# andreaskoepf/faster-rcnn.torch

Hardware: AMD Instinct MI355X
Metric: images/sec (vgg_small 800x450 fwd+bwd) (higher is better)
Workload: dtype f32 (conv / Linear(13824,1024) operands as 2 x fp16 split planes: 22 significand bits, 3 MFMA partial products; fp32 accumulate)

## Files before the change

### faster-rcnn.torch_amd/csrc/gemm.hip

```cpp
#include <cstdlib>
#include "kernels.h"

namespace frcnn {

typedef float f32x16 __attribute__((ext_vector_type(16)));

#define GB 64
#ifndef GBK
#define GBK 32
#endif

struct GemmGroup { GemmJob job[GEMM_GROUP_MAX]; int start[GEMM_GROUP_MAX + 1]; int tm[GEMM_GROUP_MAX], tn[GEMM_GROUP_MAX]; int n; };

struct GemmArgs {
  const float* A; long sAm, sAk;
  const float* B; long sBk, sBn;
  float* C; long ldc;
  const float* bias;
  int M, N, K, kPerSplit, out_mode;
};

__device__ __forceinline__ void gemm_store_tile(const f32x16& a, const GemmArgs& p, int mb, int n, int split) {
  const bool nok = n < p.N;
  const int nc = min(n, p.N - 1);
  const float bv = (p.bias && split == 0) ? p.bias[nc] : 0.f;
  float* const col = (p.out_mode == 3 ? p.C + (long)split * p.M * p.N : p.C) + nc;
  const long rs = p.out_mode == 3 ? (long)p.N : p.ldc;
  if (p.out_mode == 1) {
    float old[16];
#pragma unroll
    for (int r = 0; r < 16; ++r) old[r] = col[(long)min(mb + (r & 3) + 8 * (r >> 2), p.M - 1) * rs];
#pragma unroll
    for (int r = 0; r < 16; ++r) {
      const int m = mb + (r & 3) + 8 * (r >> 2);
      if (nok && m < p.M) col[(long)m * rs] = old[r] + (a[r] + bv);
    }
  } else {
#pragma unroll
    for (int r = 0; r < 16; ++r) {
      const int m = mb + (r & 3) + 8 * (r >> 2);
      if (nok && m < p.M) col[(long)m * rs] = a[r] + bv;
    }
  }
}


template <int ROWS, bool KC, bool VEC>
struct TileLoader {
  static constexpr int NV = ROWS * GBK / 1024;
  static constexpr int NS = ROWS * GBK / 256;
  static constexpr int PITCH = ROWS + 1;
  float4 v4[NV];
  float v1[VEC ? 1 : NS];
  __device__ __forceinline__ static void coord_v(int tid, int it, int& r, int& k) {
    if (KC) { k = (tid % (GBK / 4)) * 4; r = tid / (GBK / 4) + (1024 / GBK) * it; }
    else    { r = (tid % (ROWS / 4)) * 4; k = tid / (ROWS / 4) + (1024 / ROWS) * it; }
  }
  __device__ __forceinline__ static void coord_s(int tid, int it, int& r, int& k) {
    if (KC) { k = tid % GBK; r = tid / GBK + (256 / GBK) * it; }
    else    { r = tid % ROWS; k = tid / ROWS + (256 / ROWS) * it; }
  }
  __device__ __forceinline__ void load(const float* __restrict__ P, long sRow, long sK, int row0, int nRows, int k0,
                                       int kEnd, int tid) {
    if (VEC) {
#pragma unroll
      for (int it = 0; it < NV; ++it) {
        int r, k;
        coord_v(tid, it, r, k);
        const int rr = min(row0 + r, nRows - (KC ? 1 : 4)), kk = min(k0 + k, kEnd - (KC ? 4 : 1));
        v4[it] = *reinterpret_cast<const float4*>(P + (long)rr * sRow + (long)kk * sK);
      }
    } else {
#pragma unroll
      for (int it = 0; it < NS; ++it) {
        int r, k;
        coord_s(tid, it, r, k);
        const int rr = min(row0 + r, nRows - 1), kk = min(k0 + k, kEnd - 1);
        v1[it] = P[(long)rr * sRow + (long)kk * sK];
      }
    }
  }
  __device__ __forceinline__ void store(float* __restrict__ T, int row0, int nRows, int k0, int kEnd, int tid) {
    if (VEC) {
#pragma unroll
      for (int it = 0; it < NV; ++it) {
        int r, k;
        coord_v(tid, it, r, k);
        const float e[4] = {v4[it].x, v4[it].y, v4[it].z, v4[it].w};
#pragma unroll
        for (int j = 0; j < 4; ++j) {
          const int rj = KC ? r : r + j, kj = KC ? k + j : k;
          T[kj * PITCH + rj] = (row0 + rj < nRows && k0 + kj < kEnd) ? e[j] : 0.f;
        }
      }
    } else {
#pragma unroll
      for (int it = 0; it < NS; ++it) {
        int r, k;
        coord_s(tid, it, r, k);
        T[k * PITCH + r] = (row0 + r < nRows && k0 + k < kEnd) ? v1[it] : 0.f;
      }
    }
  }
};

template <int TM, int TN, bool AK, bool BK_, bool AV, bool BV>
__device__ __forceinline__ void gemm_tile(const GemmArgs& p, int bx, int by, int bz, float* As, float* Bs) {
  constexpr int PA = TM + 1, PB = TN + 1, MT = TM / 64, NT = TN / 64;
  const int tid = threadIdx.x, lane = tid & 63, wave = tid >> 6;
  const int wm = wave >> 1, wn = wave & 1, h = lane >> 5, li = lane & 31;
  const int m0 = by * TM, n0 = bx * TN;
  const int kbeg = bz * p.kPerSplit;
  const int kend = min(kbeg + p.kPerSplit, p.K);
  f32x16 acc[MT][NT];
#pragma unroll
  for (int a = 0; a < MT; ++a)
#pragma unroll
    for (int b = 0; b < NT; ++b)
#pragma unroll
      for (int r = 0; r < 16; ++r) acc[a][b][r] = 0.f;
  TileLoader<TM, AK, AV> la;
  TileLoader<TN, BK_, BV> lb;

  for (int k0 = kbeg; k0 < kend; k0 += GBK) {
    la.load(p.A, p.sAm, p.sAk, m0, p.M, k0, kend, tid);
    lb.load(p.B, p.sBn, p.sBk, n0, p.N, k0, kend, tid);
    la.store(As, m0, p.M, k0, kend, tid);
    lb.store(Bs, n0, p.N, k0, kend, tid);
    __syncthreads();
#pragma unroll
    for (int kk = 0; kk < GBK / 2; ++kk) {
      float a[MT], b[NT];
#pragma unroll
      for (int i = 0; i < MT; ++i) a[i] = As[(kk * 2 + h) * PA + wm * (TM / 2) + i * 32 + li];
#pragma unroll
      for (int j = 0; j < NT; ++j) b[j] = Bs[(kk * 2 + h) * PB + wn * (TN / 2) + j * 32 + li];
#pragma unroll
      for (int i = 0; i < MT; ++i)
#pragma unroll
        for (int j = 0; j < NT; ++j) acc[i][j] = __builtin_amdgcn_mfma_f32_32x32x2f32(a[i], b[j], acc[i][j], 0, 0, 0);
    }
    __syncthreads();
  }
#pragma unroll
  for (int j = 0; j < NT; ++j) {
    const int n = n0 + wn * (TN / 2) + j * 32 + li;
#pragma unroll
    for (int i = 0; i < MT; ++i)
      gemm_store_tile(acc[i][j], p, m0 + wm * (TM / 2) + i * 32 + 4 * h, n, bz);
  }
}

template <int TM, int TN, bool AK, bool BK_, bool AV, bool BV>
__global__ __launch_bounds__(256) void gemm_kernel(GemmArgs p) {
  __shared__ float As[GBK * (TM + 1)];
  __shared__ float Bs[GBK * (TN + 1)];
  gemm_tile<TM, TN, AK, BK_, AV, BV>(p, blockIdx.x, blockIdx.y, blockIdx.z, As, Bs);
}

template <bool AK, bool BK_>
__global__ __launch_bounds__(256) void gemm_group_kernel(GemmGroup g) {
  __shared__ float As[GBK * (GB + 1)];
  __shared__ float Bs[GBK * (GB + 1)];
  int j = 0;
  while (j + 1 < g.n && (int)blockIdx.x >= g.start[j + 1]) ++j;
  const int b = blockIdx.x - g.start[j];
  const int tiles = g.tn[j] * g.tm[j];
  const int bz = b / tiles, r = b - bz * tiles;
  GemmArgs p;
  const GemmJob& q = g.job[j];
  p.A = q.A; p.sAm = q.sAm; p.sAk = q.sAk; p.B = q.B; p.sBk = q.sBk; p.sBn = q.sBn; p.C = q.C; p.ldc = q.ldc; p.bias = nullptr;
  p.M = q.M; p.N = q.N; p.K = q.K; p.kPerSplit = q.kPerSplit; p.out_mode = q.out_mode;
  gemm_tile<GB, GB, AK, BK_, false, false>(p, r % g.tn[j], r / g.tn[j], bz, As, Bs);
}

#ifndef GD_BK
#define GD_BK 32
#endif
#ifndef GD_STAGES
#define GD_STAGES 1
#endif
__device__ __attribute__((aligned(16))) float g_zero16[4] = {0.f, 0.f, 0.f, 0.f};

template <int ROWS, bool KCONT>
__device__ __forceinline__ void gd_issue(const float* __restrict__ P, long sRow, long sK, int row0, int nRows, int k0,
                                         int kend, float* lds, int wave_u, int lane) {
  constexpr int NINST = ROWS * GD_BK / 256;
#pragma unroll
  for (int j = 0; j < NINST / 4; ++j) {
    const int inst = wave_u + 4 * j;
    const int slot = inst * 64 + lane;
    const float* src;
    if (KCONT) {
      const int r = slot / (GD_BK / 4), cphys = slot % (GD_BK / 4);
      const int k = k0 + ((cphys ^ (r & 7)) << 2);
      const int rr = min(row0 + r, nRows - 1);
      src = k < kend ? P + (long)rr * sRow + k : g_zero16;
    } else {
      const int kr = slot / (ROWS / 4), r4 = (slot % (ROWS / 4)) * 4;
      const int k = k0 + kr;
      const int rr = min(row0 + r4, nRows - 4);
      src = k < kend ? P + (long)k * sK + rr : g_zero16;
    }
    __builtin_amdgcn_global_load_lds((const __attribute__((address_space(1))) void*)src,
                                     (__attribute__((address_space(3))) void*)(lds + inst * 256), 16, 0, 0);
  }
}

template <int TM, int TN, bool AK, bool BK_>
__global__ __launch_bounds__(256) void gemm_dma_kernel(GemmArgs p) {
  constexpr int MT = TM / 64, NT = TN / 64;
  constexpr int AF = TM * GD_BK, BF = TN * GD_BK;
  extern __shared__ __attribute__((aligned(16))) float gsm[];
  float* As = gsm;
  float* Bs = gsm + GD_STAGES * AF;
  const int tid = threadIdx.x, lane = tid & 63;
  const int wave = __builtin_amdgcn_readfirstlane(tid >> 6);
  const int wm = wave >> 1, wn = wave & 1, h = lane >> 5, li = lane & 31;
  const int m0 = blockIdx.y * TM, n0 = blockIdx.x * TN;
  const int kbeg = blockIdx.z * p.kPerSplit;
  const int kend = min(kbeg + p.kPerSplit, p.K);
  f32x16 acc[MT][NT];
#pragma unroll
  for (int a = 0; a < MT; ++a)
#pragma unroll
    for (int b = 0; b < NT; ++b)
#pragma unroll
      for (int r = 0; r < 16; ++r) acc[a][b][r] = 0.f;

  auto stage = [&](int k0, int buf) {
    gd_issue<TM, AK>(p.A, p.sAm, p.sAk, m0, p.M, k0, kend, As + buf * AF, wave, lane);
    gd_issue<TN, BK_>(p.B, p.sBn, p.sBk, n0, p.N, k0, kend, Bs + buf * BF, wave, lane);
  };
#define GD_DMA_WAIT() asm volatile("s_waitcnt vmcnt(0)" ::: "memory")
  if (GD_STAGES == 2) stage(kbeg, 0);
  GD_DMA_WAIT();
  __syncthreads();
  int cur = 0;
  for (int k0 = kbeg; k0 < kend; k0 += GD_BK) {
    if (GD_STAGES == 2) {
      if (k0 + GD_BK < kend) stage(k0 + GD_BK, cur ^ 1);
    } else {
      stage(k0, 0);
      GD_DMA_WAIT();
      __syncthreads();
    }
    const float* A_ = As + cur * AF;
    const float* B_ = Bs + cur * BF;
#pragma unroll
    for (int g = 0; g < GD_BK / 8; ++g) {
      float a[MT][4], b[NT][4];
#pragma unroll
      for (int mt = 0; mt < MT; ++mt) {
        const int arow = wm * (TM / 2) + mt * 32 + li;
        if (AK) {
          const float4 v = *reinterpret_cast<const float4*>(A_ + (arow * (GD_BK / 4) + ((2 * g + h) ^ (arow & 7))) * 4);
          a[mt][0] = v.x; a[mt][1] = v.y; a[mt][2] = v.z; a[mt][3] = v.w;
        } else {
#pragma unroll
          for (int j = 0; j < 4; ++j) a[mt][j] = A_[(8 * g + 4 * h + j) * TM + arow];
        }
      }
#pragma unroll
      for (int nt = 0; nt < NT; ++nt) {
        const int brow = wn * (TN / 2) + nt * 32 + li;
        if (BK_) {
          const float4 v = *reinterpret_cast<const float4*>(B_ + (brow * (GD_BK / 4) + ((2 * g + h) ^ (brow & 7))) * 4);
          b[nt][0] = v.x; b[nt][1] = v.y; b[nt][2] = v.z; b[nt][3] = v.w;
        } else {
#pragma unroll
          for (int j = 0; j < 4; ++j) b[nt][j] = B_[(8 * g + 4 * h + j) * TN + brow];
        }
      }
#pragma unroll
      for (int j = 0; j < 4; ++j)
#pragma unroll
        for (int mt = 0; mt < MT; ++mt)
#pragma unroll
          for (int nt = 0; nt < NT; ++nt)
            acc[mt][nt] = __builtin_amdgcn_mfma_f32_32x32x2f32(a[mt][j], b[nt][j], acc[mt][nt], 0, 0, 0);
    }
    if (GD_STAGES == 2) GD_DMA_WAIT();
    __syncthreads();
    if (GD_STAGES == 2) cur ^= 1;
  }
#pragma unroll
  for (int j = 0; j < NT; ++j) {
    const int n = n0 + wn * (TN / 2) + j * 32 + li;
#pragma unroll
    for (int i = 0; i < MT; ++i)
      gemm_store_tile(acc[i][j], p, m0 + wm * (TM / 2) + i * 32 + 4 * h, n, (int)blockIdx.z);
  }
}

__global__ void gemm_reduce_kernel(const float* __restrict__ slab, int nSplit, int M, int N, const float* __restrict__ bias,
                                   float* __restrict__ C, long ldc, int accumulate) {
  const long total = (long)M * N;
  for (long t = (long)blockIdx.x * blockDim.x + threadIdx.x; t < total; t += (long)gridDim.x * blockDim.x) {
    const int m = (int)(t / N), n = (int)(t - (long)m * N);
    float v = bias ? bias[n] : 0.f;
    for (int sI = 0; sI < nSplit; ++sI) v += slab[(size_t)sI * total + t];
    float* dst = C + (long)m * ldc + n;
    if (accumulate) *dst += v; else *dst = v;
  }
}

static void* g_gemm_ws[8] = {};
static size_t g_gemm_ws_bytes[8] = {};
static int gemm_workspace(size_t need, float** out, int slot) {
  if (need > g_gemm_ws_bytes[slot]) {
    if (g_gemm_ws[slot]) FR_HIP(hipFree(g_gemm_ws[slot]));
    g_gemm_ws[slot] = nullptr; g_gemm_ws_bytes[slot] = 0;
    FR_HIP(hipMalloc(&g_gemm_ws[slot], need));
    g_gemm_ws_bytes[slot] = need;
  }
  *out = (float*)g_gemm_ws[slot];
  return FRCNN_OK;
}

int gemm_workspace_get(size_t need, float** out, int slot) { return gemm_workspace(need, out, slot); }
int gemm_reduce_slabs(const float* slab, int nSplit, int M, int N, const float* bias, float* C, long ldc, bool accumulate,
                      hipStream_t s) {
  const long total = (long)M * N;
  const int rgrid = (int)std::min<long>(cdivl(total, 256), 2048);
  FR_LAUNCH(KC_ELEMWISE, 0, total * 4.0 * (nSplit + 1), s, gemm_reduce_kernel, dim3(rgrid), dim3(256), 0, slab, nSplit, M, N, bias,
            C, ldc, accumulate ? 1 : 0);
  FR_LAUNCH_CHECK();
  return FRCNN_OK;
}

int gemm_f32(const float* A, long sAm, long sAk, const float* B, long sBk, long sBn, float* C,
             long ldc, int M, int N, int K, int out_mode, const float* bias_n, hipStream_t s, int ws_slot, GemmFold* defer) {
  if (defer) *defer = GemmFold{};
  if (M <= 0 || N <= 0) return FRCNN_OK;
  GemmArgs p;
  p.A = A; p.sAm = sAm; p.sAk = sAk; p.B = B; p.sBk = sBk; p.sBn = sBn; p.C = C; p.ldc = ldc;
  p.bias = bias_n; p.M = M; p.N = N; p.K = K;
  constexpr int TMs = 64;
  const int TNs = (N >= 2048 && K >= 512) ? 128 : 64;
  int tm = cdiv(M, TMs), tn = cdiv(N, TNs);
  long tiles = (long)tm * tn;
  const long slots = TNs == 128 ? 1280 : 2048;
  int splitK = (int)std::max<long>(1, std::min<long>(std::min<long>(K / 256, 16), slots / tiles));
  p.kPerSplit = cdiv(cdiv(K, splitK), GBK) * GBK;
  splitK = cdiv(K, p.kPerSplit);
  p.out_mode = out_mode;
  float* user_C = C;
  if (splitK > 1) {
    float* ws = nullptr;
    FR_TRY(gemm_workspace((size_t)splitK * M * N * 4, &ws, ws_slot & 7));
    p.C = ws; p.bias = nullptr; p.out_mode = 3;
  }
  dim3 grid(tn, tm, splitK);
  double flops = 2.0 * M * N * (double)K;
  double bytes = 4.0 * ((double)M * K + (double)K * N + (double)M * N);
  const bool ak = sAk == 1, bk = sBk == 1;
  auto vec_ok = [](const float* P, bool kc, long sRow, long sK, int nRows, int Kdim, int kPer) {
    if (((uintptr_t)P & 15) != 0) return false;
    if (kc) return sK == 1 && (sRow % 4) == 0 && (Kdim % 4) == 0 && (kPer % 4) == 0;
    return sRow == 1 && (sK % 4) == 0 && (nRows % 4) == 0;
  };
  const bool av = vec_ok(A, ak, sAm, sAk, M, K, p.kPerSplit), bv = vec_ok(B, bk, sBn, sBk, N, K, p.kPerSplit);
  auto chunk_ok = [](const float* P, bool kc, long sRow, long sK, int nRows, int Kdim, int kPer) {
    if (((uintptr_t)P & 3) != 0) return false;
    if (kc) return sK == 1 && (Kdim % 4) == 0 && (kPer % 4) == 0;
    return sRow == 1 && (nRows % 4) == 0;
  };
  const bool ad = chunk_ok(A, ak, sAm, sAk, M, K, p.kPerSplit);
  const bool bd = chunk_ok(B, bk, sBn, sBk, N, K, p.kPerSplit);
  const bool dma_ok = ad && bd && (p.kPerSplit % GD_BK == 0 || splitK == 1) && K >= 64 &&
                      (ak ? true : (M % 4 == 0 && M >= 4)) && (bk ? true : (N % 4 == 0 && N >= 4));
  if (dma_ok) {
    const size_t lds = (size_t)GD_STAGES * (TMs + TNs) * GD_BK * 4;
#define GEMM_DMA(TMv, TNv, AKv, BKv)                                                                              \
  do {                                                                                                            \
    static bool attr_ = false;                                                                                    \
    if (!attr_) {                                                                                                 \
      FR_HIP(hipFuncSetAttribute(reinterpret_cast<const void*>(gemm_dma_kernel<TMv, TNv, AKv, BKv>),              \
                                 hipFuncAttributeMaxDynamicSharedMemorySize, 160 * 1024));                        \
      attr_ = true;                                                                                               \
    }                                                                                                             \
    FR_LAUNCH(KC_GEMM, flops, bytes, s, (gemm_dma_kernel<TMv, TNv, AKv, BKv>), grid, dim3(256), lds, p);          \
  } while (0)
#define GEMM_DMA_T(TMv, TNv)                                                       \
  do {                                                                             \
    if (ak && bk) GEMM_DMA(TMv, TNv, true, true);                                  \
    else if (ak) GEMM_DMA(TMv, TNv, true, false);                                  \
    else if (bk) GEMM_DMA(TMv, TNv, false, true);                                  \
    else GEMM_DMA(TMv, TNv, false, false);                                         \
  } while (0)
    if (TNs == 128) GEMM_DMA_T(TMs, 128);
    else GEMM_DMA_T(TMs, 64);
#undef GEMM_DMA_T
#undef GEMM_DMA
  } else {
  const int sel = (ak ? 8 : 0) | (bk ? 4 : 0) | (av ? 2 : 0) | (bv ? 1 : 0);
#define GEMM_LAUNCH(TMv, TNv, AKv, BKv, AVv, BVv) \
  FR_LAUNCH(KC_GEMM, flops, bytes, s, (gemm_kernel<TMv, TNv, AKv, BKv, AVv, BVv>), grid, dim3(256), 0, p)
#define GEMM_CASE(AKv, BKv, AVv, BVv)                                                                        \
  case ((AKv ? 8 : 0) | (BKv ? 4 : 0) | (AVv ? 2 : 0) | (BVv ? 1 : 0)):                                      \
    if (TNs == 128) GEMM_LAUNCH(TMs, 128, AKv, BKv, AVv, BVv);                                               \
    else GEMM_LAUNCH(TMs, 64, AKv, BKv, AVv, BVv);                                                           \
    break;
  switch (sel) {
    GEMM_CASE(true, true, true, true) GEMM_CASE(true, true, true, false) GEMM_CASE(true, true, false, true)
    GEMM_CASE(true, true, false, false) GEMM_CASE(true, false, true, true) GEMM_CASE(true, false, true, false)
    GEMM_CASE(true, false, false, true) GEMM_CASE(true, false, false, false) GEMM_CASE(false, true, true, true)
    GEMM_CASE(false, true, true, false) GEMM_CASE(false, true, false, true) GEMM_CASE(false, true, false, false)
    GEMM_CASE(false, false, true, true) GEMM_CASE(false, false, true, false) GEMM_CASE(false, false, false, true)
    GEMM_CASE(false, false, false, false)
  }
#undef GEMM_CASE
#undef GEMM_LAUNCH
  }
  if (splitK > 1 && splitK <= 8 && defer && out_mode == OUT_STORE && ldc == N) {
    defer->slab = p.C; defer->nSplit = splitK; defer->bias = bias_n;
  } else if (splitK > 1) {
    long total = (long)M * N;
    int rgrid = (int)std::min<long>(cdivl(total, 256), 2048);
    FR_LAUNCH(KC_ELEMWISE, 0, total * 4.0 * (splitK + 1), s, gemm_reduce_kernel, dim3(rgrid), dim3(256), 0, (const float*)p.C,
              splitK, M, N, bias_n, user_C, ldc, out_mode == OUT_ADD ? 1 : 0);
  }
  FR_LAUNCH_CHECK();
  return FRCNN_OK;
}

int gemm_f32_group(GemmJob* jobs, int n, hipStream_t s) {
  FR_CHECK(n >= 1 && n <= GEMM_GROUP_MAX, "gemm_f32_group: %d jobs", n);
  GemmGroup g;
  g.n = n;
  int at = 0;
  double flops = 0, bytes = 0;
  const bool ak = jobs[0].sAk == 1, bk = jobs[0].sBk == 1;
  for (int j = 0; j < n; ++j) {
    GemmJob& q = jobs[j];
    const int splits = std::max(1, q.splits);
    q.kPerSplit = cdiv(cdiv(q.K, splits), GBK) * GBK;
    const int ns = (q.M > 0 && q.N > 0) ? cdiv(q.K, q.kPerSplit) : 0;
    if (splits > 1) { FR_CHECK(ns == splits, "gemm_f32_group: %d splits of K = %d leave one empty", splits, q.K); q.out_mode = 3; }
    g.job[j] = q;
    g.tm[j] = cdiv(q.M, GB); g.tn[j] = cdiv(q.N, GB);
    g.start[j] = at;
    at += g.tm[j] * g.tn[j] * ns;
    flops += 2.0 * q.M * q.N * (double)q.K;
    bytes += 4.0 * ((double)q.M * q.K + (double)q.K * q.N + (double)q.M * q.N);
  }
  g.start[n] = at;
  if (at == 0) return FRCNN_OK;
  if (ak && bk) FR_LAUNCH(KC_GEMM, flops, bytes, s, (gemm_group_kernel<true, true>), dim3(at), dim3(256), 0, g);
  else if (ak) FR_LAUNCH(KC_GEMM, flops, bytes, s, (gemm_group_kernel<true, false>), dim3(at), dim3(256), 0, g);
  else if (bk) FR_LAUNCH(KC_GEMM, flops, bytes, s, (gemm_group_kernel<false, true>), dim3(at), dim3(256), 0, g);
  else FR_LAUNCH(KC_GEMM, flops, bytes, s, (gemm_group_kernel<false, false>), dim3(at), dim3(256), 0, g);
  FR_LAUNCH_CHECK();
  return FRCNN_OK;
}

}
```

### faster-rcnn.torch_amd/csrc/roi.hip

```cpp
#include "kernels.h"
#include "roi_fix.h"

namespace frcnn {

__global__ void roi_pool_forward_kernel(const float* __restrict__ fmap, int C, int H, int W,
                                        const int* __restrict__ wins, int R, int kh, int kw,
                                        float* __restrict__ out, int* __restrict__ idx) {
  const long total = (long)R * C * kh * kw;
  for (long t = (long)blockIdx.x * blockDim.x + threadIdx.x; t < total; t += (long)gridDim.x * blockDim.x) {
    int j = (int)(t % kw);
    long q = t / kw;
    int i = (int)(q % kh);
    q /= kh;
    int c = (int)(q % C);
    int r = (int)(q / C);
    const int* wn = wins + 4 * r;
    const int r0 = wn[0] - 1, c0 = wn[2] - 1;
    const int h = wn[1] - wn[0] + 1, w = wn[3] - wn[2] + 1;
    const int ys = (i * h) / kh, ye = ((i + 1) * h + kh - 1) / kh;
    const int xs = (j * w) / kw, xe = ((j + 1) * w + kw - 1) / kw;
    const float* ip = fmap + (size_t)c * H * W;
    float best = -3.402823466e+38f;
    int bi = -1;
    for (int y = ys; y < ye; ++y)
      for (int x = xs; x < xe; ++x) {
        float v = ip[(size_t)(r0 + y) * W + (c0 + x)];
        if (v > best) { best = v; bi = (r0 + y) * W + (c0 + x); }
      }
    out[t] = best;
    if (idx) idx[t] = bi;
  }
}

__global__ __launch_bounds__(256) void roi_pool_forward_cells_kernel(const float* __restrict__ fmap, int C, int H, int W,
                                                                     const int* __restrict__ wins, int kh, int kw,
                                                                     float* __restrict__ out, int* __restrict__ idx) {
  const int r = blockIdx.x, cells = kh * kw, groups = blockDim.x / cells;
  const int tid = threadIdx.x;
  if (tid >= groups * cells) return;
  const int cg = tid / cells, cell = tid - cg * cells;
  const int i = cell / kw, j = cell - i * kw;
  const int* wn = wins + 4 * r;
  const int r0 = wn[0] - 1, c0 = wn[2] - 1;
  const int h = wn[1] - wn[0] + 1, w = wn[3] - wn[2] + 1;
  const int ys = (i * h) / kh, ye = ((i + 1) * h + kh - 1) / kh;
  const int xs = (j * w) / kw, xe = ((j + 1) * w + kw - 1) / kw;
  const int HW = H * W;
  const int base = (r0 + ys) * W + c0 + xs, nx = xe - xs, ny = ye - ys;
  if (HW >= 4) {
    for (int c = blockIdx.y * groups + cg; c < C; c += gridDim.y * groups) {
      const float* ip = fmap + (size_t)c * HW;
      float best = -3.402823466e+38f;
      int bi = -1;
      for (int y = 0, o = base; y < ny; ++y, o += W)
        for (int x = 0; x < nx; x += 4) {
          const int q = min(o + x, HW - 4);
          float v[4];
          __builtin_memcpy(v, ip + q, 16);
#pragma unroll
          for (int e = 0; e < 4; ++e) {
            const int at = q + e;
            if (at >= o && at < o + nx && v[e] > best) { best = v[e]; bi = at; }
          }
        }
      const size_t t = ((size_t)r * C + c) * cells + cell;
      out[t] = best;
      if (idx) idx[t] = bi;
    }
    return;
  }
  for (int c = blockIdx.y * groups + cg; c < C; c += gridDim.y * groups) {
    const float* ip = fmap + (size_t)c * HW;
    float best = -3.402823466e+38f;
    int bi = -1;
    for (int y = 0, o = base; y < ny; ++y, o += W)
      for (int x = 0; x < nx; ++x) {
        const float v = ip[o + x];
        if (v > best) { best = v; bi = o + x; }
      }
    const size_t t = ((size_t)r * C + c) * cells + cell;
    out[t] = best;
    if (idx) idx[t] = bi;
  }
}

int roi_pool_forward(const float* fmap, int C, int H, int W, const int* wins, int R, int kh, int kw,
                     float* out, int* idx, hipStream_t s) {
  if (R <= 0) return FRCNN_OK;
  long total = (long)R * C * kh * kw;
  if (kh * kw <= 256) {
    const int groups = 256 / (kh * kw);
    const int slices = std::max(1, std::min(cdiv(C, groups), (int)cdivl(4096, R)));
    FR_LAUNCH(KC_ROI, 0, total * 8.0, s, roi_pool_forward_cells_kernel, dim3(R, slices), dim3(256), 0, fmap, C, H, W,
              wins, kh, kw, out, idx);
    FR_LAUNCH_CHECK();
    return FRCNN_OK;
  }
  int grid = (int)std::min<long>(cdivl(total, 256), 4096);
  FR_LAUNCH(KC_ROI, 0, total * 8.0, s, roi_pool_forward_kernel, dim3(grid), dim3(256), 0, fmap, C, H, W,
            wins, R, kh, kw, out, idx);
  FR_LAUNCH_CHECK();
  return FRCNN_OK;
}

__global__ void roi_pool_backward_lds_kernel(float* __restrict__ gmap, int C, int HW, const float* __restrict__ gout,
                                             const int* __restrict__ idx, int R, int cell) {
  extern __shared__ float plane[];
  const int c = blockIdx.x;
  for (int i = threadIdx.x; i < HW; i += blockDim.x) plane[i] = 0.f;
  __syncthreads();
  const long D = (long)C * cell;
  const int total = R * cell;
  for (int e = threadIdx.x; e < total; e += blockDim.x) {
    const int r = e / cell, j = e - r * cell;
    const long t = (long)r * D + (long)c * cell + j;
    const int bi = idx[t];
    const float g = gout[t];
    if (bi >= 0 && g != 0.f) atomicAdd(&plane[bi], g);
  }
  __syncthreads();
  float* gp = gmap + (size_t)c * HW;
  for (int i = threadIdx.x; i < HW; i += blockDim.x) {
    const float v = plane[i];
    if (v != 0.f) gp[i] += v;
  }
}

__global__ void roi_pool_backward_lds_det_kernel(float* __restrict__ gmap, int C, int HW, const float* __restrict__ gout,
                                                 const int* __restrict__ idx, int R, int cell) {
  extern __shared__ unsigned long long fplane[];
  const int c = blockIdx.x;
  for (int i = threadIdx.x; i < HW; i += blockDim.x) fplane[i] = 0ull;
  __syncthreads();
  const long D = (long)C * cell;
  const int total = R * cell;
  for (int e = threadIdx.x; e < total; e += blockDim.x) {
    const int r = e / cell, j = e - r * cell;
    const long t = (long)r * D + (long)c * cell + j;
    const int bi = idx[t];
    const float g = gout[t];
    if (bi >= 0 && g != 0.f) atomicAdd(&fplane[bi], (unsigned long long)roi_to_fix(g));
  }
  __syncthreads();
  float* gp = gmap + (size_t)c * HW;
  for (int i = threadIdx.x; i < HW; i += blockDim.x) {
    const long long v = (long long)fplane[i];
    if (v != 0) gp[i] += (float)((double)v / ROI_FIX_SCALE);
  }
}
__global__ void roi_pool_backward_det_kernel(unsigned long long* __restrict__ fix, int C, long HW,
                                             const float* __restrict__ gout, const int* __restrict__ idx,
                                             long total, int cell) {
  for (long t = (long)blockIdx.x * blockDim.x + threadIdx.x; t < total; t += (long)gridDim.x * blockDim.x) {
    int c = (int)((t / cell) % C);
    int bi = idx[t];
    float g = gout[t];
    if (bi >= 0 && g != 0.f) atomicAdd(fix + (size_t)c * HW + bi, (unsigned long long)roi_to_fix(g));
  }
}
__global__ void roi_fix_apply_kernel(const unsigned long long* __restrict__ fix, long n, float* __restrict__ gmap) {
  for (long t = (long)blockIdx.x * blockDim.x + threadIdx.x; t < n; t += (long)gridDim.x * blockDim.x) {
    const long long v = (long long)fix[t];
    if (v != 0) gmap[t] += (float)((double)v / ROI_FIX_SCALE);
  }
}

int roi_fix_apply(const unsigned long long* fix, long n, float* gmap, hipStream_t s) {
  FR_LAUNCH(KC_ROI, 0, n * 16.0, s, roi_fix_apply_kernel, dim3((int)std::min<long>(cdivl(n, 256), 4096)), dim3(256), 0, fix, n, gmap);
  FR_LAUNCH_CHECK();
  return FRCNN_OK;
}

__global__ void roi_pool_backward_kernel(float* __restrict__ gmap, int C, long HW,
                                         const float* __restrict__ gout, const int* __restrict__ idx,
                                         long total, int cell) {
  for (long t = (long)blockIdx.x * blockDim.x + threadIdx.x; t < total; t += (long)gridDim.x * blockDim.x) {
    int c = (int)((t / cell) % C);
    int bi = idx[t];
    float g = gout[t];
    if (bi >= 0 && g != 0.f) unsafeAtomicAdd(gmap + (size_t)c * HW + bi, g);
  }
}

int roi_pool_backward(float* gmap, int C, int H, int W, const float* gout, const int* idx, int R,
                      int kh, int kw, hipStream_t s) {
  if (R <= 0) return FRCNN_OK;
  long total = (long)R * C * kh * kw;
  if (deterministic()) {
    if ((size_t)H * W * 8 <= 64 * 1024) {
      FR_LAUNCH(KC_ROI, 0, total * 12.0, s, roi_pool_backward_lds_det_kernel, dim3(C), dim3(256), (size_t)H * W * 8, gmap, C,
                H * W, gout, idx, R, kh * kw);
    } else {
      float* ws = nullptr;
      const long n = (long)C * H * W;
      FR_TRY(det_workspace(s, (size_t)n * 2, &ws));
      FR_HIP(hipMemsetAsync(ws, 0, (size_t)n * 8, s));
      int grid = (int)std::min<long>(cdivl(total, 256), 4096);
      FR_LAUNCH(KC_ROI, 0, total * 12.0, s, roi_pool_backward_det_kernel, dim3(grid), dim3(256), 0, (unsigned long long*)ws, C,
                (long)H * W, gout, idx, total, kh * kw);
      FR_LAUNCH_CHECK();
      return roi_fix_apply((const unsigned long long*)ws, n, gmap, s);
    }
    FR_LAUNCH_CHECK();
    return FRCNN_OK;
  }
  if ((size_t)H * W * 4 <= 64 * 1024) {
    FR_LAUNCH(KC_ROI, 0, total * 12.0, s, roi_pool_backward_lds_kernel, dim3(C), dim3(1024), (size_t)H * W * 4, gmap, C,
              H * W, gout, idx, R, kh * kw);
    FR_LAUNCH_CHECK();
    return FRCNN_OK;
  }
  int grid = (int)std::min<long>(cdivl(total, 256), 4096);
  FR_LAUNCH(KC_ROI, 0, total * 12.0, s, roi_pool_backward_kernel, dim3(grid), dim3(256), 0, gmap, C,
            (long)H * W, gout, idx, total, kh * kw);
  FR_LAUNCH_CHECK();
  return FRCNN_OK;
}

}
```

Before: 520.1.

## Vectorize split-K reduction and stage ROI-pool feature planes in LDS

```diff
diff --git a/faster-rcnn.torch_amd/csrc/gemm.hip b/faster-rcnn.torch_amd/csrc/gemm.hip
--- a/faster-rcnn.torch_amd/csrc/gemm.hip
+++ b/faster-rcnn.torch_amd/csrc/gemm.hip
@@ -293,16 +293,45 @@
   }
 }
 
-__global__ void gemm_reduce_kernel(const float* __restrict__ slab, int nSplit, int M, int N, const float* __restrict__ bias,
-                                   float* __restrict__ C, long ldc, int accumulate) {
-  const long total = (long)M * N;
-  for (long t = (long)blockIdx.x * blockDim.x + threadIdx.x; t < total; t += (long)gridDim.x * blockDim.x) {
-    const int m = (int)(t / N), n = (int)(t - (long)m * N);
-    float v = bias ? bias[n] : 0.f;
-    for (int sI = 0; sI < nSplit; ++sI) v += slab[(size_t)sI * total + t];
-    float* dst = C + (long)m * ldc + n;
-    if (accumulate) *dst += v; else *dst = v;
-  }
+__device__ __forceinline__ float4 gr_add(float4 a, float4 b) { return make_float4(a.x + b.x, a.y + b.y, a.z + b.z, a.w + b.w); }
+__device__ __forceinline__ float gr_add(float a, float b) { return a + b; }
+__device__ __forceinline__ void gr_zero(float4& v) { v = make_float4(0.f, 0.f, 0.f, 0.f); }
+__device__ __forceinline__ void gr_zero(float& v) { v = 0.f; }
+template <class V>
+__global__ __launch_bounds__(256) void gemm_reduce_kernel(const float* __restrict__ slab, int nSplit, int M, int N,
+                                                          const float* __restrict__ bias, float* __restrict__ C, long ldc,
+                                                          int accumulate) {
+  constexpr int E = sizeof(V) / 4;
+  const int Nv = N / E;
+  const long total = (long)M * Nv, stride = (long)gridDim.x * blockDim.x;
+  const long ldv = ldc / E;
+  const V* __restrict__ sv = reinterpret_cast<const V*>(slab);
+  const V* __restrict__ bv = reinterpret_cast<const V*>(bias);
+  V* __restrict__ cv = reinterpret_cast<V*>(C);
+  long t = (long)blockIdx.x * blockDim.x + threadIdx.x;
+  if (t >= total) return;
+  long m = t / Nv;
+  int n = (int)(t - m * Nv);
+  const long dm = stride / Nv;
+  const int dn = (int)(stride - dm * Nv);
+  for (; t < total; t += stride) {
+    V v;
+    if (bias) v = bv[n]; else gr_zero(v);
+    int sI = 0;
+    const V* p = sv + t;
+    for (; sI + 4 <= nSplit; sI += 4, p += 4 * total) {
+      const V a = p[0], b = p[total], c = p[2 * total], d = p[3 * total];
+      v = gr_add(gr_add(gr_add(gr_add(v, a), b), c), d);
+    }
+    for (; sI < nSplit; ++sI, p += total) v = gr_add(v, *p);
+    V* dst = cv + m * ldv + n;
+    *dst = accumulate ? gr_add(*dst, v) : v;
+    n += dn; m += dm;
+    if (n >= Nv) { n -= Nv; ++m; }
+  }
+}
+static bool gemm_reduce_vec_ok(const float* slab, int N, const float* bias, const float* C, long ldc) {
+  return N % 4 == 0 && ldc % 4 == 0 && (((uintptr_t)slab | (uintptr_t)bias | (uintptr_t)C) & 15) == 0;
 }
 
 static void* g_gemm_ws[8] = {};
@@ -322,9 +351,15 @@
 int gemm_reduce_slabs(const float* slab, int nSplit, int M, int N, const float* bias, float* C, long ldc, bool accumulate,
                       hipStream_t s) {
   const long total = (long)M * N;
-  const int rgrid = (int)std::min<long>(cdivl(total, 256), 2048);
-  FR_LAUNCH(KC_ELEMWISE, 0, total * 4.0 * (nSplit + 1), s, gemm_reduce_kernel, dim3(rgrid), dim3(256), 0, slab, nSplit, M, N, bias,
-            C, ldc, accumulate ? 1 : 0);
+  if (gemm_reduce_vec_ok(slab, N, bias, C, ldc)) {
+    const int rgrid = (int)std::min<long>(cdivl(total / 4, 256), 2048);
+    FR_LAUNCH(KC_ELEMWISE, 0, total * 4.0 * (nSplit + 1), s, gemm_reduce_kernel<float4>, dim3(rgrid), dim3(256), 0, slab, nSplit, M, N,
+              bias, C, ldc, accumulate ? 1 : 0);
+  } else {
+    const int rgrid = (int)std::min<long>(cdivl(total, 256), 2048);
+    FR_LAUNCH(KC_ELEMWISE, 0, total * 4.0 * (nSplit + 1), s, gemm_reduce_kernel<float>, dim3(rgrid), dim3(256), 0, slab, nSplit, M, N,
+              bias, C, ldc, accumulate ? 1 : 0);
+  }
   FR_LAUNCH_CHECK();
   return FRCNN_OK;
 }
@@ -416,10 +451,7 @@
   if (splitK > 1 && splitK <= 8 && defer && out_mode == OUT_STORE && ldc == N) {
     defer->slab = p.C; defer->nSplit = splitK; defer->bias = bias_n;
   } else if (splitK > 1) {
-    long total = (long)M * N;
-    int rgrid = (int)std::min<long>(cdivl(total, 256), 2048);
-    FR_LAUNCH(KC_ELEMWISE, 0, total * 4.0 * (splitK + 1), s, gemm_reduce_kernel, dim3(rgrid), dim3(256), 0, (const float*)p.C,
-              splitK, M, N, bias_n, user_C, ldc, out_mode == OUT_ADD ? 1 : 0);
+    FR_TRY(gemm_reduce_slabs(p.C, splitK, M, N, bias_n, user_C, ldc, out_mode == OUT_ADD, s));
   }
   FR_LAUNCH_CHECK();
   return FRCNN_OK;
diff --git a/faster-rcnn.torch_amd/csrc/roi.hip b/faster-rcnn.torch_amd/csrc/roi.hip
--- a/faster-rcnn.torch_amd/csrc/roi.hip
+++ b/faster-rcnn.torch_amd/csrc/roi.hip
@@ -84,10 +84,101 @@
   }
 }
 
+#define ROI_FWD_THREADS 512
+#define ROI_FWD_TAB 1024
+#define ROI_FWD_TAB_BYTES ((ROI_FWD_TAB + 256) * 4)
+__global__ __launch_bounds__(ROI_FWD_THREADS) void roi_pool_forward_lds_kernel(const float* __restrict__ fmap, int C, int H, int W,
+                                                                               const int* __restrict__ wins, int R, int kh, int kw,
+                                                                               int G, int rois_per_block, float* __restrict__ out,
+                                                                               int* __restrict__ idx) {
+  extern __shared__ __attribute__((aligned(16))) unsigned char roi_smem[];
+  int* const tab = reinterpret_cast<int*>(roi_smem);
+  int* const celltab = tab + ROI_FWD_TAB;
+  float* const planes = reinterpret_cast<float*>(roi_smem + ROI_FWD_TAB_BYTES);
+  const int tid = threadIdx.x, B = blockDim.x;
+  const int HW = H * W, cells = kh * kw, kk = kh + kw;
+  const int c0 = blockIdx.x * G, Gc = min(G, C - c0);
+  const int r_begin = blockIdx.y * rois_per_block, r_end = min(R, r_begin + rois_per_block);
+  {
+    const float* __restrict__ src = fmap + (size_t)c0 * HW;
+    const int n = Gc * HW;
+    int head = (int)(((16 - (reinterpret_cast<uintptr_t>(src) & 15)) & 15) >> 2);
+    if (head > n) head = n;
+    const int n4 = (n - head) >> 2;
+    const float4* __restrict__ s4 = reinterpret_cast<const float4*>(src + head);
+    for (int e = tid; e < n4; e += B) {
+      const float4 v = s4[e];
+      float* d = planes + head + 4 * e;
+      d[0] = v.x; d[1] = v.y; d[2] = v.z; d[3] = v.w;
+    }
+    if (tid < head) planes[tid] = src[tid];
+    if (head + 4 * n4 + tid < n) planes[head + 4 * n4 + tid] = src[head + 4 * n4 + tid];
+  }
+  if (tid < cells) { const int i = tid / kw; celltab[tid] = i | ((tid - i * kw) << 16); }
+  const int chunk = ROI_FWD_TAB / kk;
+  int* const ytab = tab;
+  int* const xtab = tab + chunk * kh;
+  const int d_cell = B % cells, bq = B / cells, d_cl = bq % Gc, d_rl = bq / Gc;
+  for (int rc = r_begin; rc < r_end; rc += chunk) {
+    const int nr = min(chunk, r_end - rc);
+    __syncthreads();
+    for (int e = tid; e < nr * kk; e += B) {
+      const int rl = e / kk, k = e - rl * kk;
+      const int* wn = wins + 4 * (rc + rl);
+      if (k < kh) {
+        const int r0 = wn[0] - 1, h = wn[1] - wn[0] + 1;
+        ytab[rl * kh + k] = (r0 + (k * h) / kh) | ((r0 + ((k + 1) * h + kh - 1) / kh) << 16);
+      } else {
+        const int j = k - kh, x0 = wn[2] - 1, w = wn[3] - wn[2] + 1;
+        xtab[rl * kw + j] = (x0 + (j * w) / kw) | ((x0 + ((j + 1) * w + kw - 1) / kw) << 16);
+      }
+    }
+    __syncthreads();
+    const int items = nr * Gc * cells;
+    int cell = tid % cells, q = tid / cells;
+    int cl = q % Gc, rl = q / Gc;
+    for (int t = tid; t < items; t += B) {
+      const int ij = celltab[cell], i = ij & 0xFFFF, j = ij >> 16;
+      const int yb = ytab[rl * kh + i], xb = xtab[rl * kw + j];
+      const int y0 = yb & 0xFFFF, y1 = yb >> 16, x0 = xb & 0xFFFF, x1 = xb >> 16;
+      const float* pl = planes + cl * HW;
+      float best = -3.402823466e+38f;
+      int bi = -1;
+      for (int y = y0, o = y0 * W; y < y1; ++y, o += W)
+        for (int x = x0; x < x1; ++x) {
+          const float v = pl[o + x];
+          if (v > best) { best = v; bi = o + x; }
+        }
+      const size_t at = ((size_t)(rc + rl) * C + c0 + cl) * cells + cell;
+      out[at] = best;
+      if (idx) idx[at] = bi;
+      cell += d_cell;
+      const int carry = cell >= cells;
+      cell -= carry ? cells : 0;
+      cl += d_cl + carry;
+      const int carry2 = cl >= Gc;
+      cl -= carry2 ? Gc : 0;
+      rl += d_rl + carry2;
+    }
+  }
+}
+
 int roi_pool_forward(const float* fmap, int C, int H, int W, const int* wins, int R, int kh, int kw,
                      float* out, int* idx, hipStream_t s) {
   if (R <= 0) return FRCNN_OK;
   long total = (long)R * C * kh * kw;
+  if (kh * kw <= 256 && H * W >= 4 && H <= 32767 && W <= 32767 && (size_t)H * W * 4 + ROI_FWD_TAB_BYTES <= 64 * 1024) {
+    const size_t plane = (size_t)H * W * 4;
+    int G = (int)std::max<size_t>(1, std::min<size_t>((size_t)C, (40 * 1024) / plane));
+    const int ngroups = cdiv(C, G);
+    G = cdiv(C, ngroups);
+    const int rpb = cdiv(R, std::max(1, std::min(R, 768 / ngroups)));
+    const int slices = cdiv(R, rpb);
+    FR_LAUNCH(KC_ROI, 0, total * 8.0, s, roi_pool_forward_lds_kernel, dim3(ngroups, slices), dim3(ROI_FWD_THREADS),
+              ROI_FWD_TAB_BYTES + (size_t)G * plane, fmap, C, H, W, wins, R, kh, kw, G, rpb, out, idx);
+    FR_LAUNCH_CHECK();
+    return FRCNN_OK;
+  }
   if (kh * kw <= 256) {
     const int groups = 256 / (kh * kw);
     const int slices = std::max(1, std::min(cdiv(C, groups), (int)cdivl(4096, R)));
```

Result: no change. 521.4, median of 6 (+0.2%).
